# ufukpage/TripleD-Exploring-Depth-Estimation-with-Self-Supervised-Representation-Learning

Hardware: AMD Instinct MI355X
Metric: train imgs/sec at KITTI 192x640 bs=12/GPU (higher is better)
Workload: dtype bf16 convs (MFMA) + f32 loss kernels

## Files before the change

include/tripled_hip.h:

```cpp
#ifndef TRIPLED_HIP_H
#define TRIPLED_HIP_H

#include <stddef.h>
#include <stdint.h>

#ifdef __cplusplus
extern "C" {
#endif

#define TD_ABI_VERSION 3
#define TD_MAX_SRC 4

#define TD_OK 0
#define TD_ERR_BAD_ARG (-1)
#define TD_ERR_UNSUPPORTED (-2)
#define TD_ERR_LAUNCH (-3)
#define TD_ERR_WORKSPACE (-4)

typedef void* td_stream_t;

int td_abi_version(void);
const char* td_error_string(int code);
const char* td_last_hip_error(void);

// ... 113 lines not shown

int td_bn_partial_rows(long long M, int groups, int C);
int td_bn_fwd_partials(const void* x, int dtype, long long M, int groups, int C, float* partials, td_stream_t stream);
int td_bn_bwd_partials(const void* dy, const void* x, const void* y, int dtype, const float* gamma, const float* beta,
                       const float* save_mean, const float* save_invstd, int relu, long long M, int groups, int C, float* partials,
                       td_stream_t stream);
int td_bn_bwd_from_partials(const void* dy, const void* x, const void* y, int dtype, const float* gamma, const float* beta,
                            const float* save_mean, const float* save_invstd, int relu, long long M, int groups, int C,
                            float* partials, int stat_rows, void* dx, void* dresidual, float* dgamma, float* dbeta,
                            td_stream_t stream);
int td_conv1x1_fwd_bnrelu(const void* z, const void* w, long long M, int groups, int K, int N, float* in_partials, int in_rows,
                          const float* gamma, const float* beta, float* running_mean, float* running_var, float momentum, float eps,
                          float* save_mean, float* save_invstd, void* a_side, void* y, float* stat_partials, td_stream_t stream);
int td_conv1x1_dgrad(const void* dy, const void* w, long long M, int groups, int Cout, int Cin, const void* residual, void* dx,
                     td_stream_t stream);
int td_conv1x1_fwd_sum(const void* x, const void* w, long long M, int K, int N, const void* run_in, void* y, void* run_out,
                       td_stream_t stream);
int td_conv1x1_dgrad_bnsums(const void* dy, const void* w, long long M, int groups, int Cout, int Cin, const void* z,
                            const float* gamma, const float* beta, const float* save_mean, const float* save_invstd, void* dx,
                            float* out_partials, td_stream_t stream);
int td_conv1x1_dgrad_bnbwd(const void* g, const void* z, const void* w, long long M, int groups, int Cout, int Cin, float* in_partials,
                           int in_rows, const float* gamma, const float* beta, const float* save_mean, const float* save_invstd,
                           float* dgamma, float* dbeta, void* dz_side, const void* residual, void* dx, td_stream_t stream);

int td_bn_sync_fwd_sums(const void* x, int dtype, long long M, int groups, int C, float* sums, float* workspace,
                        td_stream_t stream);
int td_bn_sync_fwd_apply(const void* x, const void* residual, int dtype, const float* sums, const float* count,
                         const float* gamma, const float* beta, float* running_mean, float* running_var, float momentum,
                         float eps, int relu, long long M, int groups, int C, void* y, float* save_mean,
                         float* save_invstd, td_stream_t stream);
int td_bn_sync_bwd_sums(const void* dy, const void* x, const void* y, int dtype, const float* gamma, const float* beta,
                        const float* save_mean, const float* save_invstd, int relu, long long M, int groups, int C,
                        float* sums, float* workspace, td_stream_t stream);
int td_bn_sync_bwd_dx(const void* dy, const void* x, const void* y, int dtype, const float* local_sums,
                      const float* global_sums, const float* count, const float* gamma, const float* beta,
                      const float* save_mean, const float* save_invstd, int relu, long long M, int groups, int C,
                      void* dx, void* dresidual, float* dgamma, float* dbeta, float* coef, td_stream_t stream);

int td_edge_weights(const float* img, int B, int h, int w, float a, const float* scale6, float* Wt,
                    td_stream_t stream);
int td_featreg_num_blocks(int B, int h, int w, int C);
int td_featreg_fwd(const void* feat, int dtype, const float* Wt, int B, int h, int w, int C,
                   float* partial, td_stream_t stream);
int td_featreg_bwd(const void* feat, int dtype, const float* Wt, const float* gscale, int B, int h, int w,
                   int C, void* grad, td_stream_t stream);

// ... 106 lines not shown
```

tripled-exploring-depth-estimation-with-self-supervised-representation-learning_amd/csrc/td_conv1x1.hip:

```cpp
#include "td_conv_tile.h"

namespace td {

struct ConvRows {
  int Wo, HoWo, Wi, HiWi, stride;
};

__device__ __forceinline__ long long cv_src_row(long long m, const ConvRows& g) {
  if (g.stride == 1) return m;
  const long long b = m / g.HoWo;
  const int rem = (int)(m - b * g.HoWo);
  const int ho = rem / g.Wo, wo = rem - ho * g.Wo;
  return b * g.HiWi + (long long)ho * g.stride * g.Wi + (long long)wo * g.stride;
}

struct CvFuse {
  const __hip_bfloat16* a2;
  const float* part;
  int part_S, part_stride, part_rows;
  const float* gamma;
  const float* beta;
  float* mean;
  float* invstd;
  float* rmean;
// ... 33 lines not shown
    g0 = fmaf(z0, sc[2 * e], sh[2 * e]) <= 0.f ? 0.f : g0;
    g1 = fmaf(z1, sc[2 * e + 1], sh[2 * e + 1]) <= 0.f ? 0.f : g1;
    const float v0 = fmaf(k0[2 * e], g0, fmaf(k1[2 * e], z0, k2[2 * e]));
    const float v1 = fmaf(k0[2 * e + 1], g1, fmaf(k1[2 * e + 1], z1, k2[2 * e + 1]));
    o[e] = (unsigned)f2bf(v0) | ((unsigned)f2bf(v1) << 16);
  }
  return make_uint4(o[0], o[1], o[2], o[3]);
}

__device__ __forceinline__ void cv_sum_rows(const float* __restrict__ part, int S, int stride, int K, int c, float& A, float& B) {
  float2 v[CV_PRO_MAX_S];
#pragma unroll
  for (int u = 0; u < CV_PRO_MAX_S; ++u)
    v[u] = *reinterpret_cast<const float2*>(part + ((size_t)(u < S ? u : 0) * stride * K + c) * 2);
  A = 0.f;
  B = 0.f;
#pragma unroll
  for (int u = 0; u < CV_PRO_MAX_S; ++u) {
    A += u < S ? v[u].x : 0.f;
    B += u < S ? v[u].y : 0.f;
  }
}

template <int BM, int BN, bool BT, int PRO, int EPI, bool DEEP>
__global__ __launch_bounds__(CV_THREADS, 2) void conv1x1_mfma_kernel(
    const __hip_bfloat16* __restrict__ x, const __hip_bfloat16* __restrict__ w, __hip_bfloat16* __restrict__ y,
    float* __restrict__ ws, long long Mg, int K, int N, int tiles_per_group, int total_blocks, ConvRows geom, CvFuse fz) {
  using T = CvTile<BM, BN, BT>;
  constexpr int A_BYTES = T::A_BYTES, STAGE = T::STAGE, TN = T::TN, TM = T::TM;
  __shared__ __attribute__((aligned(16))) unsigned char lds[T::LDS_BYTES];
  __shared__ __attribute__((aligned(16))) float s_pro[PRO == 0 ? 4 : (PRO == 1 ? 2 : 5) * CV_PRO_MAX_K];

  const int tid = threadIdx.x, lane = tid & 63, wid = tid >> 6;
  const int wm = wid >> 1, wn = wid & 1, l31 = lane & 31, h = lane >> 5;

  const int L = cv_xcd_tile(blockIdx.x, total_blocks);
  const int NT = N / BN;
  const int nt = L % NT, mt = L / NT;
  const int grp = mt / tiles_per_group, s = mt - grp * tiles_per_group;
  const long long row0 = (long long)grp * Mg + (long long)s * BM;
  const int rows_valid = (int)((Mg - (long long)s * BM) < BM ? (Mg - (long long)s * BM) : BM);
  const int n0 = nt * BN;

  const int lc = tid & 7, lr = tid >> 3;
  constexpr int NA = BM / 32, NB = BN / 32;
  auto a_off = [&](int i) {
    int r = lr + 32 * i;
    r = r < rows_valid ? r : rows_valid - 1;
    return cv_src_row(row0 + r, geom) * (long long)K + lc * 8;
  };
  const long long oa0 = a_off(0), oa1 = a_off(1), oa2 = NA > 2 ? a_off(2) : oa0, oa3 = NA > 2 ? a_off(3) : oa0;
  const __hip_bfloat16 *pa0 = x + oa0, *pa1 = x + oa1, *pa2 = x + oa2, *pa3 = x + oa3;
  constexpr int CPR = BN / 8, RPP = CV_THREADS / CPR;
  const int bc = tid % CPR, br = tid / CPR;
  const __hip_bfloat16* pb0 = BT ? w + (long long)br * N + n0 + bc * 8 : w + (long long)(n0 + lr) * K + lc * 8;
  const long long bstep = BT ? (long long)RPP * N : 32ll * K;
  const __hip_bfloat16 *pb1 = pb0 + bstep, *pb2 = pb0 + (NB > 2 ? 2 : 0) * bstep, *pb3 = pb0 + (NB > 2 ? 3 : 0) * bstep;
  const long long bkt = BT ? (long long)CV_BK * N : (long long)CV_BK;
#define CV_DECL(S)                                                                          \
  uint4 ra0##S, ra1##S, ra2##S, ra3##S, rb0##S, rb1##S, rb2##S, rb3##S, rz0##S, rz1##S, rz2##S, rz3##S; \
  ra0##S = ra1##S = ra2##S = ra3##S = rb0##S = rb1##S = rb2##S = rb3##S = make_uint4(0, 0, 0, 0);       \
  rz0##S = rz1##S = rz2##S = rz3##S = make_uint4(0, 0, 0, 0);
  CV_DECL(A)
  CV_DECL(B)
#define CV_LD(p, kt) (*reinterpret_cast<const uint4*>((p) + (kt) * CV_BK))
#define CV_LDB(p, kt) (*reinterpret_cast<const uint4*>((p) + (kt) * bkt))
#define CV_LOAD_GLOBAL(kt, S)                                  \
  {                                                            \
    ra0##S = CV_LD(pa0, kt);                                   \
    ra1##S = CV_LD(pa1, kt);                                   \
    if (NA > 2) { ra2##S = CV_LD(pa2, kt); ra3##S = CV_LD(pa3, kt); } \
    if constexpr (PRO == 2) {                                  \
      rz0##S = CV_LD(fz.a2 + oa0, kt);                         \
      rz1##S = CV_LD(fz.a2 + oa1, kt);                         \
      if (NA > 2) { rz2##S = CV_LD(fz.a2 + oa2, kt); rz3##S = CV_LD(fz.a2 + oa3, kt); } \
    }                                                          \
    rb0##S = CV_LDB(pb0, kt);                                  \
    rb1##S = CV_LDB(pb1, kt);                                  \
    if (NB > 2) { rb2##S = CV_LDB(pb2, kt); rb3##S = CV_LDB(pb3, kt); } \
  }
#define CV_ST(base, i, v) (*reinterpret_cast<uint4*>((base) + cv_swz(lr + 32 * (i), lc)) = (v))
#define CV_STB(base, i, v)                                                                              \
  {                                                                                                     \
    if constexpr (BT) *reinterpret_cast<uint4*>((base) + (br + RPP * (i)) * T::PITCH_T + bc * 16) = (v); \
    else CV_ST(base, i, v);                                                                             \
  }
#define CV_PRO_A(kt, S)                                                                                 \
// ... 32 lines not shown
  }
#define CV_WRITE_LDS(stage, kt, S)                                       \
  {                                                                      \
    unsigned char* base_ = lds + (stage) * STAGE;                        \
    CV_PRO_A(kt, S)                                                      \
    CV_ST(base_, 0, ra0##S);                                             \
    CV_ST(base_, 1, ra1##S);                                             \
    if (NA > 2) { CV_ST(base_, 2, ra2##S); CV_ST(base_, 3, ra3##S); }    \
    CV_STB(base_ + A_BYTES, 0, rb0##S);                                  \
    CV_STB(base_ + A_BYTES, 1, rb1##S);                                  \
    if (NB > 2) { CV_STB(base_ + A_BYTES, 2, rb2##S); CV_STB(base_ + A_BYTES, 3, rb3##S); } \
  }

  CvAcc<BM, BN> acc;
#pragma unroll
  for (int i = 0; i < TN; ++i)
#pragma unroll
    for (int j = 0; j < TM; ++j)
#pragma unroll
      for (int e = 0; e < 16; ++e) acc.v[i][j][e] = 0.f;

  const int nk = K / CV_BK;
  CV_LOAD_GLOBAL(0, A)
  if constexpr (DEEP) CV_LOAD_GLOBAL(nk > 1 ? 1 : 0, B)

  if constexpr (PRO == 1) {
    const float* part = fz.part + (size_t)grp * fz.part_rows * K * 2;
    const bool first = (s == 0 && nt == 0);
    for (int c = tid; c < K; c += CV_THREADS) {
      float A, B;
      cv_sum_rows(part, fz.part_S, fz.part_stride, K, c, A, B);
      const double m = (double)A / (double)Mg;
      double var = (double)B / (double)Mg - m * m;
      var = var > 0.0 ? var : 0.0;
      const float mf = (float)m, isf = (float)(1.0 / sqrt(var + (double)fz.eps));
      const float scv = fz.gamma[c] * isf;
      s_pro[c] = scv;
      s_pro[CV_PRO_MAX_K + c] = fz.beta[c] - mf * scv;
      if (first) {
        fz.mean[(size_t)grp * K + c] = mf;
        fz.invstd[(size_t)grp * K + c] = isf;
      }
      if (fz.rmean && first && grp == 0) {
        double rm = fz.rmean[c], rv = fz.rvar[c];
        for (int g2 = 0; g2 < fz.G; ++g2) {
          float A2 = A, B2 = B;
          if (g2 != 0) cv_sum_rows(fz.part + (size_t)g2 * fz.part_rows * K * 2, fz.part_S, fz.part_stride, K, c, A2, B2);
// ... 23 lines not shown
      const float c1 = -c0 * is * dg * inv_m;
      s_pro[0 * CV_PRO_MAX_K + c] = c0;
      s_pro[1 * CV_PRO_MAX_K + c] = c1;
      s_pro[2 * CV_PRO_MAX_K + c] = -c0 * A * inv_m - c1 * mu;
      s_pro[3 * CV_PRO_MAX_K + c] = c0;
      s_pro[4 * CV_PRO_MAX_K + c] = fz.beta[c] - mu * c0;
      if (first) {
        float dg_tot = 0.f, db_tot = 0.f;
        for (int g2 = 0; g2 < fz.G; ++g2) {
          float A2 = A, B2 = B;
          if (g2 != 0) cv_sum_rows(fz.part + (size_t)g2 * fz.part_rows * K * 2, fz.part_S, fz.part_stride, K, c, A2, B2);
          dg_tot += B2 * fz.invstd[(size_t)g2 * K + c];
          db_tot += A2;
        }
        fz.dgamma[c] = dg_tot;
        fz.dbeta[c] = db_tot;
      }
    }
    __syncthreads();
  }

  CV_WRITE_LDS(0, 0, A)
  __syncthreads();
  if constexpr (!DEEP) {
    for (int kt = 0; kt < nk; ++kt) {
      const bool more = kt + 1 < nk;
      if (more) CV_LOAD_GLOBAL(kt + 1, A)
      const unsigned char* sa = lds + (kt & 1) * STAGE;
      cv_stage_mfma<BM, BN, BT>(acc, sa, sa + A_BYTES, wm, wn, l31, h);
      if (more) CV_WRITE_LDS((kt + 1) & 1, kt + 1, A)
      __syncthreads();
    }
  } else {
    const int last = nk - 1;
    for (int kt = 0; kt < nk; kt += 2) {
      const int k2 = kt + 2 < last ? kt + 2 : last, k1 = kt + 1 < last ? kt + 1 : last, k3 = kt + 3 < last ? kt + 3 : last;
      CV_LOAD_GLOBAL(k2, A)
      __builtin_amdgcn_sched_barrier(0);
      cv_stage_mfma<BM, BN, BT>(acc, lds, lds + A_BYTES, wm, wn, l31, h);
      CV_WRITE_LDS(1, k1, B)
      __syncthreads();
      if (kt + 1 >= nk) break;
      CV_LOAD_GLOBAL(k3, B)
      __builtin_amdgcn_sched_barrier(0);
      cv_stage_mfma<BM, BN, BT>(acc, lds + STAGE, lds + STAGE + A_BYTES, wm, wn, l31, h);
      CV_WRITE_LDS(0, k2, A)
      __syncthreads();
    }
  }

  CvEpi ep = fz.ep;
  if constexpr (EPI == 2) { ep.mean += (size_t)grp * N; ep.invstd += (size_t)grp * N; }
  cv_epilogue<BM, BN, EPI>(acc, lds, y, ws, row0, rows_valid, n0, N, (long long)grp * tiles_per_group + s, tid, wm, wn, l31, h, ep);
}

#undef CV_LOAD_GLOBAL
#undef CV_DECL
#undef CV_WRITE_LDS
#undef CV_PRO_A
#undef CV_LD
#undef CV_LDB
#undef CV_ST
#undef CV_STB

constexpr int WG_T = 64;
constexpr int WG_PITCH = WG_T * 2 + 64;

typedef __attribute__((ext_vector_type(4))) short cv_s16x4;

__device__ __forceinline__ cv_bf16x8 wg_frag(const unsigned char* tile, int col0, int ks, int lane) {
  const int g = lane >> 4, i = lane & 15;
  const int row = 16 * ks + 8 * (g >> 1) + (i >> 2);
  const unsigned char* p = tile + row * WG_PITCH + (col0 + 16 * (g & 1) + 4 * (i & 3)) * 2;
  typedef __attribute__((address_space(3))) cv_s16x4* lds_ptr;
  const cv_s16x4 lo = __builtin_amdgcn_ds_read_tr16_b64_v4i16((lds_ptr)(p));
  const cv_s16x4 hi = __builtin_amdgcn_ds_read_tr16_b64_v4i16((lds_ptr)(p + 4 * WG_PITCH));
  typedef __attribute__((ext_vector_type(8))) short s16x8;
  const s16x8 v = {lo[0], lo[1], lo[2], lo[3], hi[0], hi[1], hi[2], hi[3]};
  return __builtin_bit_cast(cv_bf16x8, v);
}

constexpr int WG_TILE_BYTES = WG_T * WG_PITCH, WG_STAGE = 2 * WG_TILE_BYTES, WG_LDS_BYTES = 2 * WG_STAGE;

__device__ __forceinline__ void wgrad_block(
    const __hip_bfloat16* __restrict__ dy, const __hip_bfloat16* __restrict__ x, float* __restrict__ part, long long M, int K, int N,
    int rows_per_split, int tiles_n, int tiles_k, ConvRows geom, int L, unsigned char* lds) {
  constexpr int TILE_BYTES = WG_TILE_BYTES, STAGE = WG_STAGE;
  const int tid = threadIdx.x, lane = tid & 63, wid = tid >> 6;
  const int wn = wid >> 1, wk = wid & 1;
  const int nt = L % tiles_n, kt = (L / tiles_n) % tiles_k, sp = L / (tiles_n * tiles_k);
  const int n0 = nt * WG_T, k0 = kt * WG_T;
  const long long m_lo = (long long)sp * rows_per_split;
  const long long m_hi = (m_lo + rows_per_split < M) ? m_lo + rows_per_split : M;
  const int nstage = (int)((m_hi - m_lo + WG_T - 1) / WG_T);

  const int lc = tid & 7, lr = tid >> 3;
  uint4 ry0a, ry1a, rx0a, rx1a, ry0b, ry1b, rx0b, rx1b;
#define WG_LOAD(st, S)                                                                                             \
  {                                                                                                                \
    const long long r0 = m_lo + (long long)(st) * WG_T + lr, r1 = r0 + 32;                                         \
    const uint4 z = make_uint4(0, 0, 0, 0);                                                                        \
    ry0##S = r0 < m_hi ? *reinterpret_cast<const uint4*>(dy + r0 * N + n0 + lc * 8) : z;                           \
    ry1##S = r1 < m_hi ? *reinterpret_cast<const uint4*>(dy + r1 * N + n0 + lc * 8) : z;                           \
    rx0##S = r0 < m_hi ? *reinterpret_cast<const uint4*>(x + cv_src_row(r0, geom) * (long long)K + k0 + lc * 8) : z; \
    rx1##S = r1 < m_hi ? *reinterpret_cast<const uint4*>(x + cv_src_row(r1, geom) * (long long)K + k0 + lc * 8) : z; \
  }
#define WG_WRITE(buf, S)                                                                         \
  {                                                                                              \
    unsigned char* b_ = lds + (buf) * STAGE;                                                     \
    *reinterpret_cast<uint4*>(b_ + lr * WG_PITCH + lc * 16) = ry0##S;                            \
    *reinterpret_cast<uint4*>(b_ + (lr + 32) * WG_PITCH + lc * 16) = ry1##S;                     \
    *reinterpret_cast<uint4*>(b_ + TILE_BYTES + lr * WG_PITCH + lc * 16) = rx0##S;               \
    *reinterpret_cast<uint4*>(b_ + TILE_BYTES + (lr + 32) * WG_PITCH + lc * 16) = rx1##S;        \
  }
#define WG_MFMA(buf)                                                                             \
  {                                                                                              \
    const unsigned char* ty = lds + (buf) * STAGE;                                               \
    const unsigned char* tx = ty + TILE_BYTES;                                                   \
    _Pragma("unroll") for (int ks = 0; ks < WG_T / 16; ++ks) {                                   \
      const cv_bf16x8 fa = wg_frag(ty, wn * 32, ks, lane);                  \
      const cv_bf16x8 fb = wg_frag(tx, wk * 32, ks, lane);                  \
      acc = __builtin_amdgcn_mfma_f32_32x32x16_bf16(fa, fb, acc, 0, 0, 0);                       \
    }                                                                                            \
  }
  cv_f32x16 acc;
#pragma unroll
  for (int e = 0; e < 16; ++e) acc[e] = 0.f;
  WG_LOAD(0, a)
  if (nstage > 1) WG_LOAD(1, b)
  WG_WRITE(0, a)
  __syncthreads();
  for (int st = 0; st < nstage; st += 2) {
    if (st + 2 < nstage) WG_LOAD(st + 2, a)
    WG_MFMA(0)
    if (st + 1 < nstage) WG_WRITE(1, b)
    __syncthreads();
    if (st + 1 >= nstage) break;
    if (st + 3 < nstage) WG_LOAD(st + 3, b)
    WG_MFMA(1)
    if (st + 2 < nstage) WG_WRITE(0, a)
    __syncthreads();
  }
#undef WG_MFMA
#undef WG_LOAD
#undef WG_WRITE
  float* out = part + ((size_t)sp * N + n0 + wn * 32 + 4 * (lane >> 5)) * K + k0 + wk * 32 + (lane & 31);
#pragma unroll
  for (int r = 0; r < 16; ++r) out[(size_t)((r & 3) + 8 * (r >> 2)) * K] = acc[r];
}

__global__ __launch_bounds__(CV_THREADS, 2) void conv1x1_wgrad_kernel(
    const __hip_bfloat16* __restrict__ dy, const __hip_bfloat16* __restrict__ x, float* __restrict__ part, long long M, int K, int N,
    int rows_per_split, int tiles_n, int tiles_k, ConvRows geom) {
  __shared__ __attribute__((aligned(16))) unsigned char lds[WG_LDS_BYTES];
  wgrad_block(dy, x, part, M, K, N, rows_per_split, tiles_n, tiles_k, geom, cv_xcd_tile(blockIdx.x, gridDim.x), lds);
}

constexpr int WG_GROUP_MAX = 40;
struct WgProblem {
  const __hip_bfloat16* dy;
  const __hip_bfloat16* x;
  float* part;
  long long M;
  int K, N, rows_per_split, tiles_n, tiles_k;
  ConvRows geom;
};
struct WgGroupArgs {
  WgProblem p[WG_GROUP_MAX];
  int first_block[WG_GROUP_MAX + 1];
  int n;
};
__global__ __launch_bounds__(CV_THREADS, 2) void conv1x1_wgrad_group_kernel(const WgGroupArgs a) {
  __shared__ __attribute__((aligned(16))) unsigned char lds[WG_LDS_BYTES];
  const int L = cv_xcd_tile(blockIdx.x, gridDim.x);
  int lo = 0, hi = a.n;
  while (hi - lo > 1) {
    const int mid = (lo + hi) >> 1;
    if (a.first_block[mid] <= L) lo = mid; else hi = mid;
  }
  const WgProblem& q = a.p[lo];
  wgrad_block(q.dy, q.x, q.part, q.M, q.K, q.N, q.rows_per_split, q.tiles_n, q.tiles_k, q.geom, L - a.first_block[lo], lds);
}

template <typename T>
__global__ __launch_bounds__(TD_THREADS) void conv1x1_wgrad_reduce_kernel(const float* __restrict__ part, int P, long long NK, T* __restrict__ dw) {
  __shared__ float4 red[16][16];
  const int c = threadIdx.x & 15, g = threadIdx.x >> 4;
  const long long i = ((long long)blockIdx.x * 16 + c) * 4;
  float4 a = make_float4(0.f, 0.f, 0.f, 0.f);
  if (i < NK) {
    for (int p = g; p < P; p += 16) {
      const float4 b = *reinterpret_cast<const float4*>(part + (size_t)p * NK + i);
      a.x += b.x; a.y += b.y; a.z += b.z; a.w += b.w;
    }
  }
  red[g][c] = a;
  __syncthreads();
  if (g == 0 && i < NK) {
#pragma unroll
    for (int j = 1; j < 16; ++j) {
      const float4 b = red[j][c];
      a.x += b.x; a.y += b.y; a.z += b.z; a.w += b.w;
    }
    if constexpr (sizeof(T) == 2) {
// ... 54 lines not shown
      *reinterpret_cast<float4*>(reinterpret_cast<float*>(q.dw) + i) = s4;
    }
  }
}

int cv_wgrad_reduce(const float* part, int P, long long NK, int dw_dtype, void* dw, hipStream_t st) {
  const unsigned blocks = (unsigned)((NK / 4 + 15) / 16);
  if (dw_dtype == TD_DTYPE_BF16)
    hipLaunchKernelGGL((conv1x1_wgrad_reduce_kernel<__hip_bfloat16>), dim3(blocks), dim3(TD_THREADS), 0, st, part, P, NK, (__hip_bfloat16*)dw);
  else
    hipLaunchKernelGGL((conv1x1_wgrad_reduce_kernel<float>), dim3(blocks), dim3(TD_THREADS), 0, st, part, P, NK, (float*)dw);
  return hipGetLastError() == hipSuccess ? TD_OK : TD_ERR_LAUNCH;
}

static inline int wg_splits(long long M, int K, int N) {
  const long long tiles = (long long)(N / WG_T) * (K / WG_T);
  long long p = (768 + tiles - 1) / tiles;
  const long long by_rows = (M + 4 * WG_T - 1) / (4 * WG_T);
  if (p > by_rows) p = by_rows;
  if (p > 512) p = 512;
  return (int)(p < 1 ? 1 : p);
}

template <int BM, int BN, bool BT, int PRO, int EPI, bool DEEP>
static int cv_launch(const void* x, const void* w, void* y, float* ws, long long Mg, int G, int K, int N, ConvRows geom, hipStream_t st,
                     const CvFuse& fz) {
  const int tpg = (int)((Mg + BM - 1) / BM);
  const long long nblk = (long long)G * tpg * (N / BN);
  if (nblk > 0x7fffffffll) return TD_ERR_UNSUPPORTED;
  hipLaunchKernelGGL((conv1x1_mfma_kernel<BM, BN, BT, PRO, EPI, DEEP>), dim3((unsigned)nblk), dim3(CV_THREADS), 0, st, (const __hip_bfloat16*)x,
                     (const __hip_bfloat16*)w, (__hip_bfloat16*)y, ws, Mg, K, N, tpg, (int)nblk, geom, fz);
  return hipGetLastError() == hipSuccess ? TD_OK : TD_ERR_LAUNCH;
}

template <bool BT, int PRO, int EPI>
static int cv_dispatch(const void* x, const void* w, void* y, float* ws, long long M, int G, int K, int N, ConvRows geom, hipStream_t st,
                       const CvFuse& fz) {
  const long long Mg = M / G;
  ConvTile t = cv_pick_tile(Mg, G, N);
  const bool deep = K >= 3 * CV_BK;
  if constexpr (PRO == 2) {
    if (t.bm == 128 && t.bn == 128) t.bn = 64;
  } else
    if (t.bm == 128 && t.bn == 128) return cv_launch<128, 128, BT, PRO, EPI, false>(x, w, y, ws, Mg, G, K, N, geom, st, fz);
  if (t.bm == 128 && t.bn == 64) {
    if constexpr (PRO == 0)
      if (deep) return cv_launch<128, 64, BT, PRO, EPI, true>(x, w, y, ws, Mg, G, K, N, geom, st, fz);
    return cv_launch<128, 64, BT, PRO, EPI, false>(x, w, y, ws, Mg, G, K, N, geom, st, fz);
  }
  if (deep) return cv_launch<64, 64, BT, PRO, EPI, true>(x, w, y, ws, Mg, G, K, N, geom, st, fz);
  return cv_launch<64, 64, BT, PRO, EPI, false>(x, w, y, ws, Mg, G, K, N, geom, st, fz);
}

}

static bool cv_shape_ok(long long M, int G, int K, int N) {
  return M > 0 && G >= 1 && G <= 64 && M % G == 0 && K > 0 && N > 0 && K % 64 == 0 && N % 64 == 0;
}

extern "C" int td_conv1x1_stat_rows(long long M, int groups, int N) {
  if (M <= 0 || groups < 1 || M % groups != 0 || N <= 0 || N % 64 != 0) return 0;
  const td::ConvTile t = td::cv_pick_tile(M / groups, groups, N);
  return (int)((M / groups + t.bm - 1) / t.bm);
}

extern "C" int td_conv1x1_fwd(const void* x, const void* w, long long M, int groups, int K, int N, int Hi, int Wi, int stride, void* y,
                              float* stat_partials, td_stream_t stream) {
  if (!x || !w || !y || !cv_shape_ok(M, groups, K, N) || stride < 1) return TD_ERR_BAD_ARG;
  td::ConvRows geom = {0, 0, 0, 0, 1};
  if (stride > 1) {
    if (Hi <= 0 || Wi <= 0) return TD_ERR_BAD_ARG;
    const int Ho = (Hi - 1) / stride + 1, Wo = (Wi - 1) / stride + 1;
    if (M % ((long long)Ho * Wo) != 0) return TD_ERR_BAD_ARG;
    geom = {Wo, Ho * Wo, Wi, Hi * Wi, stride};
  }
  if (M * (long long)(K > N ? K : N) >= (1ll << 40)) return TD_ERR_UNSUPPORTED;
  return td::cv_dispatch<false, 0, 0>(x, w, y, stat_partials, M, groups, K, N, geom, (hipStream_t)stream, td::CvFuse{});
}

namespace td {
// ... 72 lines not shown
extern "C" long long td_conv1x1_wgrad_workspace_floats(long long M, int K, int N) {
  if (M <= 0 || K <= 0 || N <= 0 || K % 64 != 0 || N % 64 != 0) return 0;
  return (long long)td::wg_splits(M, K, N) * N * K;
}

extern "C" int td_conv1x1_wgrad(const void* dy, const void* x, long long M, int K, int N, int Hi, int Wi, int stride, int dw_dtype,
                                void* dw, float* workspace, td_stream_t stream) {
  if (!dy || !x || !dw || !workspace || M <= 0 || K <= 0 || N <= 0 || K % 64 != 0 || N % 64 != 0 || stride < 1) return TD_ERR_BAD_ARG;
  if (dw_dtype != TD_DTYPE_BF16 && dw_dtype != TD_DTYPE_F32) return TD_ERR_UNSUPPORTED;
  td::ConvRows geom = {0, 0, 0, 0, 1};
  if (stride > 1) {
    if (Hi <= 0 || Wi <= 0) return TD_ERR_BAD_ARG;
    const int Ho = (Hi - 1) / stride + 1, Wo = (Wi - 1) / stride + 1;
    if (M % ((long long)Ho * Wo) != 0) return TD_ERR_BAD_ARG;
    geom = {Wo, Ho * Wo, Wi, Hi * Wi, stride};
  }
  if (M * (long long)(K > N ? K : N) >= (1ll << 40)) return TD_ERR_UNSUPPORTED;
  hipStream_t st = (hipStream_t)stream;
  const int P = td::wg_splits(M, K, N);
  long long rps = (M + P - 1) / P;
  rps = (rps + td::WG_T - 1) / td::WG_T * td::WG_T;
  const int P_eff = (int)((M + rps - 1) / rps);
  const int tn = N / td::WG_T, tk = K / td::WG_T;
  hipLaunchKernelGGL(td::conv1x1_wgrad_kernel, dim3((unsigned)(tn * tk * P_eff)), dim3(td::CV_THREADS), 0, st, (const __hip_bfloat16*)dy,
                     (const __hip_bfloat16*)x, workspace, M, K, N, (int)rps, tn, tk, geom);
  const long long NK = (long long)N * K;
  const unsigned blocks = (unsigned)((NK / 4 + 15) / 16);
  if (dw_dtype == TD_DTYPE_BF16)
    hipLaunchKernelGGL((td::conv1x1_wgrad_reduce_kernel<__hip_bfloat16>), dim3(blocks), dim3(TD_THREADS), 0, st, (const float*)workspace, P_eff,
                       NK, (__hip_bfloat16*)dw);
  else
    hipLaunchKernelGGL((td::conv1x1_wgrad_reduce_kernel<float>), dim3(blocks), dim3(TD_THREADS), 0, st, (const float*)workspace, P_eff, NK,
                       (float*)dw);
  return hipGetLastError() == hipSuccess ? TD_OK : TD_ERR_LAUNCH;
}

extern "C" int td_conv1x1_wgrad_group(int n, const void* const* dy, const void* const* x, const long long* M, const int* K, const int* N,
                                      const int* Hi, const int* Wi, const int* stride, const int* dw_dtype, void* const* dw,
                                      float* const* workspace, td_stream_t stream) {
  if (n < 0 || (n > 0 && (!dy || !x || !M || !K || !N || !Hi || !Wi || !stride || !dw_dtype || !dw || !workspace))) return TD_ERR_BAD_ARG;
  hipStream_t st = (hipStream_t)stream;
  for (int i = 0; i < n; ++i) {
    if (!dy[i] || !x[i] || !dw[i] || !workspace[i] || M[i] <= 0 || K[i] <= 0 || N[i] <= 0 || K[i] % 64 != 0 || N[i] % 64 != 0 || stride[i] < 1)
      return TD_ERR_BAD_ARG;
    if (dw_dtype[i] != TD_DTYPE_BF16 && dw_dtype[i] != TD_DTYPE_F32) return TD_ERR_UNSUPPORTED;
    if (M[i] * (long long)(K[i] > N[i] ? K[i] : N[i]) >= (1ll << 40)) return TD_ERR_UNSUPPORTED;
    if (stride[i] > 1) {
      if (Hi[i] <= 0 || Wi[i] <= 0) return TD_ERR_BAD_ARG;
      const int Ho = (Hi[i] - 1) / stride[i] + 1, Wo = (Wi[i] - 1) / stride[i] + 1;
      if (M[i] % ((long long)Ho * Wo) != 0) return TD_ERR_BAD_ARG;
    }
  }
  int P_eff[4096];
  if (n > 4096) return TD_ERR_UNSUPPORTED;
  for (int base = 0; base < n; base += td::WG_GROUP_MAX) {
    td::WgGroupArgs a;
    a.n = n - base < td::WG_GROUP_MAX ? n - base : td::WG_GROUP_MAX;
    long long blocks = 0;
    for (int j = 0; j < a.n; ++j) {
      const int i = base + j;
      td::ConvRows geom = {0, 0, 0, 0, 1};
      if (stride[i] > 1) {
        const int Ho = (Hi[i] - 1) / stride[i] + 1, Wo = (Wi[i] - 1) / stride[i] + 1;
        geom = {Wo, Ho * Wo, Wi[i], Hi[i] * Wi[i], stride[i]};
      }
      const int P = td::wg_splits(M[i], K[i], N[i]);
      long long rps = (M[i] + P - 1) / P;
      rps = (rps + td::WG_T - 1) / td::WG_T * td::WG_T;
      P_eff[i] = (int)((M[i] + rps - 1) / rps);
      td::WgProblem& q = a.p[j];
      q.dy = (const __hip_bfloat16*)dy[i]; q.x = (const __hip_bfloat16*)x[i]; q.part = workspace[i]; q.M = M[i]; q.K = K[i]; q.N = N[i];
      q.rows_per_split = (int)rps; q.tiles_n = N[i] / td::WG_T; q.tiles_k = K[i] / td::WG_T; q.geom = geom;
      a.first_block[j] = (int)blocks;
      blocks += (long long)q.tiles_n * q.tiles_k * P_eff[i];
      if (blocks > 0x7fffffffll) return TD_ERR_UNSUPPORTED;
    }
    for (int j = a.n; j <= td::WG_GROUP_MAX; ++j) a.first_block[j] = (int)blocks;
    hipLaunchKernelGGL(td::conv1x1_wgrad_group_kernel, dim3((unsigned)blocks), dim3(td::CV_THREADS), 0, st, a);
  }
  for (int base = 0; base < n; base += td::RD_GROUP_MAX) {
    td::RdGroupArgs a;
    a.n = n - base < td::RD_GROUP_MAX ? n - base : td::RD_GROUP_MAX;
    long long blocks = 0;
    for (int j = 0; j < a.n; ++j) {
      const int i = base + j;
      td::RdProblem& q = a.p[j];
      q.part = workspace[i]; q.dw = dw[i]; q.NK = (long long)N[i] * K[i]; q.P = P_eff[i]; q.bf16 = dw_dtype[i] == TD_DTYPE_BF16;
      a.first_block[j] = (int)blocks;
      blocks += (q.NK / 4 + 15) / 16;
    }
    for (int j = a.n; j <= td::RD_GROUP_MAX; ++j) a.first_block[j] = (int)blocks;
    hipLaunchKernelGGL(td::conv1x1_wgrad_reduce_group_kernel, dim3((unsigned)blocks), dim3(TD_THREADS), 0, st, a);
  }
  return hipGetLastError() == hipSuccess ? TD_OK : TD_ERR_LAUNCH;
}
```

tripled-exploring-depth-estimation-with-self-supervised-representation-learning_amd/native.py:

```python
import ctypes
import os

import torch

from . import dispatch

_HERE = os.path.dirname(os.path.abspath(__file__))
LIB_PATH = os.path.join(_HERE, "lib", "libtripled_hip.so")

TD_MAX_SRC = 4

_PTRARR = ctypes.POINTER(ctypes.c_void_p)
_I, _F, _P = ctypes.c_int, ctypes.c_float, ctypes.c_void_p
_LLARR = ctypes.POINTER(ctypes.c_longlong)
_IARR = ctypes.POINTER(ctypes.c_int)
ABI_VERSION = 3

SIGNATURES = {
    "td_abi_version": (_I, []),
    "td_error_string": (ctypes.c_char_p, [_I]),
    "td_last_hip_error": (ctypes.c_char_p, []),
    "td_photo_num_blocks": (_I, [_I, _I, _I]),
    "td_photo_bwd_num_blocks": (_I, [_I, _I, _I]),
    "td_photo_identity": (_I, [_P, _PTRARR, _I, _I, _I, _I, _P, _P, _PTRARR, _P]),
# ... 23 lines not shown
    "td_bn_fwd": (_I, [_P, _P, _I, _P, _P, _P, _P, _F, _F, _I, ctypes.c_longlong, _I, _I, _P, _P, _P, _P, _P]),
    "td_conv1x1_stat_rows": (_I, [ctypes.c_longlong, _I, _I]),
    "td_conv1x1_fwd": (_I, [_P, _P, ctypes.c_longlong, _I, _I, _I, _I, _I, _I, _P, _P, _P]),
    "td_conv3x3_fwd": (_I, [_P, _P, _I, _I, _I, _I, _I, _I, _I, _I, _P, _P, _P]),
    "td_conv3x3_wgrad_workspace_floats": (ctypes.c_longlong, [_I, _I, _I, _I, _I]),
    "td_conv3x3_wgrad": (_I, [_P, _P, _I, _I, _I, _I, _I, _I, _I, _P, _P, _P]),
    "td_conv1x1_wgrad_workspace_floats": (ctypes.c_longlong, [ctypes.c_longlong, _I, _I]),
    "td_conv1x1_wgrad": (_I, [_P, _P, ctypes.c_longlong, _I, _I, _I, _I, _I, _I, _P, _P, _P]),
    "td_conv1x1_wgrad_group": (_I, [_I, _PTRARR, _PTRARR, _LLARR, _IARR, _IARR, _IARR, _IARR, _IARR, _IARR, _PTRARR, _PTRARR, _P]),
    "td_bn_fwd_from_partials": (_I, [_P, _P, _I, _P, _P, _P, _P, _F, _F, _I, ctypes.c_longlong, _I, _I, _P, _I, _P, _P, _P, _P]),
    "td_bias_act_workspace_floats": (ctypes.c_longlong, [ctypes.c_longlong, _I]),
    "td_bias_act_fwd": (_I, [_P, _P, _I, _I, ctypes.c_longlong, _I, _I, _P, _P]),
    "td_bias_act_bwd": (_I, [_P, _P, _I, ctypes.c_longlong, _I, _I, _P, _P, _I, _P, _P]),
    "td_gather_flat": (_I, [_PTRARR, _LLARR, _LLARR, _I, _I, _P, _P]),
    "td_adam_flat": (_I, [_P, _P, _P, _P, _P, ctypes.c_longlong, ctypes.c_longlong, _P, _P, _F, ctypes.c_double, ctypes.c_double, _F, _P, _F, _P]),
    "td_bn_partial_rows": (_I, [ctypes.c_longlong, _I, _I]),
    "td_bn_fwd_partials": (_I, [_P, _I, ctypes.c_longlong, _I, _I, _P, _P]),
    "td_bn_bwd_partials": (_I, [_P, _P, _P, _I, _P, _P, _P, _P, _I, ctypes.c_longlong, _I, _I, _P, _P]),
    "td_bn_bwd_from_partials": (_I, [_P, _P, _P, _I, _P, _P, _P, _P, _I, ctypes.c_longlong, _I, _I, _P, _I, _P, _P, _P, _P, _P]),
    "td_conv1x1_fwd_bnrelu": (_I, [_P, _P, ctypes.c_longlong, _I, _I, _I, _P, _I, _P, _P, _P, _P, _F, _F, _P, _P, _P, _P, _P, _P]),
    "td_conv1x1_dgrad": (_I, [_P, _P, ctypes.c_longlong, _I, _I, _I, _P, _P, _P]),
    "td_conv1x1_dgrad_bnsums": (_I, [_P, _P, ctypes.c_longlong, _I, _I, _I, _P, _P, _P, _P, _P, _P, _P, _P]),
    "td_conv1x1_dgrad_bnbwd": (_I, [_P, _P, _P, ctypes.c_longlong, _I, _I, _I, _P, _I, _P, _P, _P, _P, _P, _P, _P, _P, _P, _P]),
    "td_bn_bwd": (_I, [_P, _P, _P, _I, _P, _P, _P, _P, _I, ctypes.c_longlong, _I, _I, _P, _P, _P, _P, _P, _P]),
    "td_edge_weights": (_I, [_P, _I, _I, _I, _F, ctypes.POINTER(ctypes.c_float), _P, _P]),
    "td_featreg_num_blocks": (_I, [_I, _I, _I, _I]),
    "td_featreg_fwd": (_I, [_P, _I, _P, _I, _I, _I, _I, _P, _P]),
    "td_featreg_bwd": (_I, [_P, _I, _P, _P, _I, _I, _I, _I, _P, _P]),
    "td_recon_num_tasks": (_I, [_I, _I, _I]),
    "td_recon_fwd": (_I, [_P, _P, _P, _I, _I, _I, _P, _P]),
    "td_recon_bwd": (_I, [_P, _P, _P, _P, _I, _I, _I, _P, _P]),
    "td_reflpad1_fwd": (_I, [_P, _I, _I, _I, _I, _I, _P, _P]),
    "td_reflpad1_bwd": (_I, [_P, _I, _I, _I, _I, _I, _P, _P]),
    "td_up2_reflpad1_fwd": (_I, [_P, _I, _I, _I, _I, _I, _P, _P]),
    "td_up2_reflpad1_bwd": (_I, [_P, _I, _I, _I, _I, _I, _P, _P]),
    "td_featwarp_num_blocks": (_I, [_I, _I, _I]),
    "td_featwarp_fwd": (_I, [_P, _PTRARR, _I, _I, _P, _P, _P, _I, _I, _I, _I, _I, _I, _F, _F, _P, _P, _P]),
    "td_featwarp_bwd": (_I, [_P, _PTRARR, _I, _I, _P, _P, _P, _P, _P, _F, _I, _I, _I, _I, _I, _I, _F, _F, _P, _PTRARR,
                             _P, _P, _P]),
    "td_featwarp_dsrc_finish": (_I, [_P, _P, _F, _I, ctypes.c_longlong, _I, _P, _P]),
    "td_reduce_partials": (_I, [_P, _I, _I, _I, _P, _P]),
    "td_bn_sync_fwd_sums": (_I, [_P, _I, ctypes.c_longlong, _I, _I, _P, _P, _P]),
    "td_bn_sync_fwd_apply": (_I, [_P, _P, _I, _P, _P, _P, _P, _P, _P, _F, _F, _I, ctypes.c_longlong, _I, _I, _P, _P, _P, _P]),
    "td_bn_sync_bwd_sums": (_I, [_P, _P, _P, _I, _P, _P, _P, _P, _I, ctypes.c_longlong, _I, _I, _P, _P, _P]),
    "td_bn_sync_bwd_dx": (_I, [_P, _P, _P, _I, _P, _P, _P, _P, _P, _P, _P, _I, ctypes.c_longlong, _I, _I, _P, _P, _P, _P, _P, _P]),
    "td_fp8_num_blocks": (_I, [ctypes.c_longlong]),
# ... 151 lines not shown
```

Baseline: 444.5.

## Add depth-4 global-load prefetch pipeline to 1x1 conv forward and wgrad kernels

Generalises the 1x1 conv MFMA kernel's prefetch from a boolean deep mode to a depth template (1, 2 or 4). A four-register-stage rotation keeps more global loads in flight ahead of the MFMA stages. Depth 4 is chosen for 64x64 tiles with long K and few blocks, and for wgrad kernels with enough output tiles; an env var and API cap allow overriding. The aim is to hide memory latency in low-occupancy, long-K convolutions, at the cost of more live registers (risking spills or lower occupancy) and extra template instantiations.

```diff
diff --git a/include/tripled_hip.h b/include/tripled_hip.h
--- a/include/tripled_hip.h
+++ b/include/tripled_hip.h
@@ -159,6 +159,8 @@
 int td_conv1x1_dgrad_bnbwd(const void* g, const void* z, const void* w, long long M, int groups, int Cout, int Cin, float* in_partials,
                            int in_rows, const float* gamma, const float* beta, const float* save_mean, const float* save_invstd,
                            float* dgamma, float* dbeta, void* dz_side, const void* residual, void* dx, td_stream_t stream);
+#define TD_CONV1X1_DEPTH_FORCE 0x100
+int td_conv1x1_prefetch_depth(int cap);
 
 int td_bn_sync_fwd_sums(const void* x, int dtype, long long M, int groups, int C, float* sums, float* workspace,
                         td_stream_t stream);
diff --git a/tripled-exploring-depth-estimation-with-self-supervised-representation-learning_amd/csrc/td_conv1x1.hip b/tripled-exploring-depth-estimation-with-self-supervised-representation-learning_amd/csrc/td_conv1x1.hip
--- a/tripled-exploring-depth-estimation-with-self-supervised-representation-learning_amd/csrc/td_conv1x1.hip
+++ b/tripled-exploring-depth-estimation-with-self-supervised-representation-learning_amd/csrc/td_conv1x1.hip
@@ -1,3 +1,6 @@
+#include <atomic>
+#include <cstdlib>
+
 #include "td_conv_tile.h"
 
 namespace td {
@@ -79,7 +82,7 @@
   }
 }
 
-template <int BM, int BN, bool BT, int PRO, int EPI, bool DEEP>
+template <int BM, int BN, bool BT, int PRO, int EPI, int DEPTH>
 __global__ __launch_bounds__(CV_THREADS, 2) void conv1x1_mfma_kernel(
     const __hip_bfloat16* __restrict__ x, const __hip_bfloat16* __restrict__ w, __hip_bfloat16* __restrict__ y,
     float* __restrict__ ws, long long Mg, int K, int N, int tiles_per_group, int total_blocks, ConvRows geom, CvFuse fz) {
@@ -120,6 +123,8 @@
   rz0##S = rz1##S = rz2##S = rz3##S = make_uint4(0, 0, 0, 0);
   CV_DECL(A)
   CV_DECL(B)
+  CV_DECL(C)
+  CV_DECL(D)
 #define CV_LD(p, kt) (*reinterpret_cast<const uint4*>((p) + (kt) * CV_BK))
 #define CV_LDB(p, kt) (*reinterpret_cast<const uint4*>((p) + (kt) * bkt))
 #define CV_LOAD_GLOBAL(kt, S)                                  \
@@ -198,7 +203,11 @@
 
   const int nk = K / CV_BK;
   CV_LOAD_GLOBAL(0, A)
-  if constexpr (DEEP) CV_LOAD_GLOBAL(nk > 1 ? 1 : 0, B)
+  if constexpr (DEPTH >= 2) CV_LOAD_GLOBAL(nk > 1 ? 1 : 0, B)
+  if constexpr (DEPTH == 4) {
+    CV_LOAD_GLOBAL(nk > 2 ? 2 : nk - 1, C)
+    CV_LOAD_GLOBAL(nk > 3 ? 3 : nk - 1, D)
+  }
 
   if constexpr (PRO == 1) {
     const float* part = fz.part + (size_t)grp * fz.part_rows * K * 2;
@@ -268,7 +277,7 @@
 
   CV_WRITE_LDS(0, 0, A)
   __syncthreads();
-  if constexpr (!DEEP) {
+  if constexpr (DEPTH == 1) {
     for (int kt = 0; kt < nk; ++kt) {
       const bool more = kt + 1 < nk;
       if (more) CV_LOAD_GLOBAL(kt + 1, A)
@@ -277,7 +286,7 @@
       if (more) CV_WRITE_LDS((kt + 1) & 1, kt + 1, A)
       __syncthreads();
     }
-  } else {
+  } else if constexpr (DEPTH == 2) {
     const int last = nk - 1;
     for (int kt = 0; kt < nk; kt += 2) {
       const int k2 = kt + 2 < last ? kt + 2 : last, k1 = kt + 1 < last ? kt + 1 : last, k3 = kt + 3 < last ? kt + 3 : last;
@@ -293,6 +302,37 @@
       CV_WRITE_LDS(0, k2, A)
       __syncthreads();
     }
+  } else {
+    static_assert(DEPTH == 4, "prefetch depth is 1, 2 or 4");
+    const int last = nk - 1;
+#define CV_STEP(i, SL, SW)                                                                          \
+  {                                                                                                  \
+    const int kl_ = kt + (i) + 4 < last ? kt + (i) + 4 : last, kw_ = kt + (i) + 1 < last ? kt + (i) + 1 : last; \
+    CV_LOAD_GLOBAL(kl_, SL)                                                                          \
+    __builtin_amdgcn_sched_barrier(0);                                                               \
+    cv_stage_mfma<BM, BN, BT>(acc, lds + ((i) & 1) * STAGE, lds + ((i) & 1) * STAGE + A_BYTES, wm, wn, l31, h); \
+    __builtin_amdgcn_sched_barrier(0);                                                               \
+    CV_WRITE_LDS(((i) + 1) & 1, kw_, SW)                                                             \
+    __syncthreads();                                                                                 \
+    __builtin_amdgcn_sched_barrier(0);                                                               \
+  }
+    int kt = 0;
+    {
+      for (; kt + 4 <= nk; kt += 4) {
+        CV_STEP(0, A, B)
+        CV_STEP(1, B, C)
+        CV_STEP(2, C, D)
+        CV_STEP(3, D, A)
+      }
+      if (kt < nk) {
+        CV_STEP(0, A, B)
+        if (kt + 1 < nk) {
+          CV_STEP(1, B, C)
+          if (kt + 2 < nk) CV_STEP(2, C, D)
+        }
+      }
+    }
+#undef CV_STEP
   }
 
   CvEpi ep = fz.ep;
@@ -326,8 +366,11 @@
   return __builtin_bit_cast(cv_bf16x8, v);
 }
 
+__device__ __forceinline__ uint4 wg_keep(uint4 v, unsigned mask) { return make_uint4(v.x & mask, v.y & mask, v.z & mask, v.w & mask); }
+
 constexpr int WG_TILE_BYTES = WG_T * WG_PITCH, WG_STAGE = 2 * WG_TILE_BYTES, WG_LDS_BYTES = 2 * WG_STAGE;
 
+template <int DEPTH>
 __device__ __forceinline__ void wgrad_block(
     const __hip_bfloat16* __restrict__ dy, const __hip_bfloat16* __restrict__ x, float* __restrict__ part, long long M, int K, int N,
     int rows_per_split, int tiles_n, int tiles_k, ConvRows geom, int L, unsigned char* lds) {
@@ -372,20 +415,65 @@
   cv_f32x16 acc;
 #pragma unroll
   for (int e = 0; e < 16; ++e) acc[e] = 0.f;
-  WG_LOAD(0, a)
-  if (nstage > 1) WG_LOAD(1, b)
-  WG_WRITE(0, a)
-  __syncthreads();
-  for (int st = 0; st < nstage; st += 2) {
-    if (st + 2 < nstage) WG_LOAD(st + 2, a)
-    WG_MFMA(0)
-    if (st + 1 < nstage) WG_WRITE(1, b)
+  if constexpr (DEPTH == 2) {
+    WG_LOAD(0, a)
+    if (nstage > 1) WG_LOAD(1, b)
+    WG_WRITE(0, a)
     __syncthreads();
-    if (st + 1 >= nstage) break;
-    if (st + 3 < nstage) WG_LOAD(st + 3, b)
-    WG_MFMA(1)
-    if (st + 2 < nstage) WG_WRITE(0, a)
+    for (int st = 0; st < nstage; st += 2) {
+      if (st + 2 < nstage) WG_LOAD(st + 2, a)
+      WG_MFMA(0)
+      if (st + 1 < nstage) WG_WRITE(1, b)
+      __syncthreads();
+      if (st + 1 >= nstage) break;
+      if (st + 3 < nstage) WG_LOAD(st + 3, b)
+      WG_MFMA(1)
+      if (st + 2 < nstage) WG_WRITE(0, a)
+      __syncthreads();
+    }
+  } else {
+    static_assert(DEPTH == 4, "prefetch depth is 2 or 4");
+    uint4 ry0c, ry1c, rx0c, rx1c, ry0d, ry1d, rx0d, rx1d;
+#define WG_LOAD4(st, S)                                                                                            \
+  {                                                                                                                \
+    const long long r0 = m_lo + (long long)(st) * WG_T + lr, r1 = r0 + 32;                                         \
+    const long long c0 = r0 < m_hi ? r0 : m_hi - 1, c1 = r1 < m_hi ? r1 : m_hi - 1;                                \
+    const unsigned k0_ = r0 < m_hi ? 0xffffffffu : 0u, k1_ = r1 < m_hi ? 0xffffffffu : 0u;                         \
+    ry0##S = wg_keep(*reinterpret_cast<const uint4*>(dy + c0 * N + n0 + lc * 8), k0_);                             \
+    ry1##S = wg_keep(*reinterpret_cast<const uint4*>(dy + c1 * N + n0 + lc * 8), k1_);                             \
+    rx0##S = wg_keep(*reinterpret_cast<const uint4*>(x + cv_src_row(c0, geom) * (long long)K + k0 + lc * 8), k0_); \
+    rx1##S = wg_keep(*reinterpret_cast<const uint4*>(x + cv_src_row(c1, geom) * (long long)K + k0 + lc * 8), k1_); \
+  }
+#define WG_STEP4(i, SL, SW)                         \
+  {                                                 \
+    WG_LOAD4(st + (i) + 4, SL)                      \
+    __builtin_amdgcn_sched_barrier(0);              \
+    WG_MFMA((i) & 1)                                \
+    WG_WRITE(((i) + 1) & 1, SW)                     \
+    __syncthreads();                                \
+  }
+    WG_LOAD4(0, a)
+    WG_LOAD4(1, b)
+    WG_LOAD4(2, c)
+    WG_LOAD4(3, d)
+    WG_WRITE(0, a)
     __syncthreads();
+    int st = 0;
+    for (; st + 4 <= nstage; st += 4) {
+      WG_STEP4(0, a, b)
+      WG_STEP4(1, b, c)
+      WG_STEP4(2, c, d)
+      WG_STEP4(3, d, a)
+    }
+    if (st < nstage) {
+      WG_STEP4(0, a, b)
+      if (st + 1 < nstage) {
+        WG_STEP4(1, b, c)
+        if (st + 2 < nstage) WG_STEP4(2, c, d)
+      }
+    }
+#undef WG_STEP4
+#undef WG_LOAD4
   }
 #undef WG_MFMA
 #undef WG_LOAD
@@ -395,11 +483,12 @@
   for (int r = 0; r < 16; ++r) out[(size_t)((r & 3) + 8 * (r >> 2)) * K] = acc[r];
 }
 
+template <int DEPTH>
 __global__ __launch_bounds__(CV_THREADS, 2) void conv1x1_wgrad_kernel(
     const __hip_bfloat16* __restrict__ dy, const __hip_bfloat16* __restrict__ x, float* __restrict__ part, long long M, int K, int N,
     int rows_per_split, int tiles_n, int tiles_k, ConvRows geom) {
   __shared__ __attribute__((aligned(16))) unsigned char lds[WG_LDS_BYTES];
-  wgrad_block(dy, x, part, M, K, N, rows_per_split, tiles_n, tiles_k, geom, cv_xcd_tile(blockIdx.x, gridDim.x), lds);
+  wgrad_block<DEPTH>(dy, x, part, M, K, N, rows_per_split, tiles_n, tiles_k, geom, cv_xcd_tile(blockIdx.x, gridDim.x), lds);
 }
 
 constexpr int WG_GROUP_MAX = 40;
@@ -409,6 +498,7 @@
   float* part;
   long long M;
   int K, N, rows_per_split, tiles_n, tiles_k;
+  int depth;
   ConvRows geom;
 };
 struct WgGroupArgs {
@@ -416,6 +506,7 @@
   int first_block[WG_GROUP_MAX + 1];
   int n;
 };
+template <int DEPTH>
 __global__ __launch_bounds__(CV_THREADS, 2) void conv1x1_wgrad_group_kernel(const WgGroupArgs a) {
   __shared__ __attribute__((aligned(16))) unsigned char lds[WG_LDS_BYTES];
   const int L = cv_xcd_tile(blockIdx.x, gridDim.x);
@@ -425,7 +516,10 @@
     if (a.first_block[mid] <= L) lo = mid; else hi = mid;
   }
   const WgProblem& q = a.p[lo];
-  wgrad_block(q.dy, q.x, q.part, q.M, q.K, q.N, q.rows_per_split, q.tiles_n, q.tiles_k, q.geom, L - a.first_block[lo], lds);
+  if (DEPTH == 4 && q.depth == 4)
+    wgrad_block<4>(q.dy, q.x, q.part, q.M, q.K, q.N, q.rows_per_split, q.tiles_n, q.tiles_k, q.geom, L - a.first_block[lo], lds);
+  else
+    wgrad_block<2>(q.dy, q.x, q.part, q.M, q.K, q.N, q.rows_per_split, q.tiles_n, q.tiles_k, q.geom, L - a.first_block[lo], lds);
 }
 
 template <typename T>
@@ -526,15 +620,40 @@
   return (int)(p < 1 ? 1 : p);
 }
 
-template <int BM, int BN, bool BT, int PRO, int EPI, bool DEEP>
+template <int BM, int BN, bool BT, int PRO, int EPI, int DEPTH>
 static int cv_launch(const void* x, const void* w, void* y, float* ws, long long Mg, int G, int K, int N, ConvRows geom, hipStream_t st,
                      const CvFuse& fz) {
   const int tpg = (int)((Mg + BM - 1) / BM);
   const long long nblk = (long long)G * tpg * (N / BN);
   if (nblk > 0x7fffffffll) return TD_ERR_UNSUPPORTED;
-  hipLaunchKernelGGL((conv1x1_mfma_kernel<BM, BN, BT, PRO, EPI, DEEP>), dim3((unsigned)nblk), dim3(CV_THREADS), 0, st, (const __hip_bfloat16*)x,
+  hipLaunchKernelGGL((conv1x1_mfma_kernel<BM, BN, BT, PRO, EPI, DEPTH>), dim3((unsigned)nblk), dim3(CV_THREADS), 0, st, (const __hip_bfloat16*)x,
                      (const __hip_bfloat16*)w, (__hip_bfloat16*)y, ws, Mg, K, N, tpg, (int)nblk, geom, fz);
   return hipGetLastError() == hipSuccess ? TD_OK : TD_ERR_LAUNCH;
+}
+
+static bool cv_depth_cap_ok(int cap) { return cap == 0 || cap == 1 || cap == 2 || cap == 4 || cap == (4 | TD_CONV1X1_DEPTH_FORCE); }
+static std::atomic<int>& cv_depth_cap() {
+  static std::atomic<int> cap{[] {
+    const char* e = getenv("TD_CONV1X1_DEPTH");
+    const int v = e ? atoi(e) : 0;
+    return cv_depth_cap_ok(v) ? v : 0;
+  }()};
+  return cap;
+}
+constexpr int CV_D4_MIN_NK = 32, CV_D4_MAX_BLOCKS = 256;
+static int cv_depth(int bm, int pro, int nk, long long blocks) {
+  int d = nk >= 3 ? 2 : 1;
+  if (bm == 128 && pro != 0) d = 1;
+  const int cap = cv_depth_cap().load(std::memory_order_relaxed);
+  if (bm == 64 && pro == 0 && (cap == (4 | TD_CONV1X1_DEPTH_FORCE) || (nk >= CV_D4_MIN_NK && blocks <= CV_D4_MAX_BLOCKS))) d = 4;
+  if (cap == 1 || cap == 2) d = d < cap ? d : cap;
+  return d;
+}
+static int wg_depth(int K, int N) {
+  const int cap = cv_depth_cap().load(std::memory_order_relaxed);
+  if (cap == 1 || cap == 2) return 2;
+  if (cap == (4 | TD_CONV1X1_DEPTH_FORCE)) return 4;
+  return (long long)(N / WG_T) * (K / WG_T) >= 16 ? 4 : 2;
 }
 
 template <bool BT, int PRO, int EPI>
@@ -542,24 +661,31 @@
                        const CvFuse& fz) {
   const long long Mg = M / G;
   ConvTile t = cv_pick_tile(Mg, G, N);
-  const bool deep = K >= 3 * CV_BK;
   if constexpr (PRO == 2) {
     if (t.bm == 128 && t.bn == 128) t.bn = 64;
   } else
-    if (t.bm == 128 && t.bn == 128) return cv_launch<128, 128, BT, PRO, EPI, false>(x, w, y, ws, Mg, G, K, N, geom, st, fz);
+    if (t.bm == 128 && t.bn == 128) return cv_launch<128, 128, BT, PRO, EPI, 1>(x, w, y, ws, Mg, G, K, N, geom, st, fz);
+  const int depth = cv_depth(t.bm, PRO, K / CV_BK, (long long)G * ((Mg + t.bm - 1) / t.bm) * (N / t.bn));
   if (t.bm == 128 && t.bn == 64) {
     if constexpr (PRO == 0)
-      if (deep) return cv_launch<128, 64, BT, PRO, EPI, true>(x, w, y, ws, Mg, G, K, N, geom, st, fz);
-    return cv_launch<128, 64, BT, PRO, EPI, false>(x, w, y, ws, Mg, G, K, N, geom, st, fz);
-  }
-  if (deep) return cv_launch<64, 64, BT, PRO, EPI, true>(x, w, y, ws, Mg, G, K, N, geom, st, fz);
-  return cv_launch<64, 64, BT, PRO, EPI, false>(x, w, y, ws, Mg, G, K, N, geom, st, fz);
+      if (depth == 2) return cv_launch<128, 64, BT, PRO, EPI, 2>(x, w, y, ws, Mg, G, K, N, geom, st, fz);
+    return cv_launch<128, 64, BT, PRO, EPI, 1>(x, w, y, ws, Mg, G, K, N, geom, st, fz);
+  }
+  if constexpr (PRO == 0)
+    if (depth == 4) return cv_launch<64, 64, BT, PRO, EPI, 4>(x, w, y, ws, Mg, G, K, N, geom, st, fz);
+  if (depth == 2) return cv_launch<64, 64, BT, PRO, EPI, 2>(x, w, y, ws, Mg, G, K, N, geom, st, fz);
+  return cv_launch<64, 64, BT, PRO, EPI, 1>(x, w, y, ws, Mg, G, K, N, geom, st, fz);
 }
 
 }
 
 static bool cv_shape_ok(long long M, int G, int K, int N) {
   return M > 0 && G >= 1 && G <= 64 && M % G == 0 && K > 0 && N > 0 && K % 64 == 0 && N % 64 == 0;
+}
+
+extern "C" int td_conv1x1_prefetch_depth(int cap) {
+  if (!td::cv_depth_cap_ok(cap)) return TD_ERR_BAD_ARG;
+  return td::cv_depth_cap().exchange(cap);
 }
 
 extern "C" int td_conv1x1_stat_rows(long long M, int groups, int N) {
@@ -678,8 +804,12 @@
   rps = (rps + td::WG_T - 1) / td::WG_T * td::WG_T;
   const int P_eff = (int)((M + rps - 1) / rps);
   const int tn = N / td::WG_T, tk = K / td::WG_T;
-  hipLaunchKernelGGL(td::conv1x1_wgrad_kernel, dim3((unsigned)(tn * tk * P_eff)), dim3(td::CV_THREADS), 0, st, (const __hip_bfloat16*)dy,
-                     (const __hip_bfloat16*)x, workspace, M, K, N, (int)rps, tn, tk, geom);
+  if (td::wg_depth(K, N) == 4)
+    hipLaunchKernelGGL(td::conv1x1_wgrad_kernel<4>, dim3((unsigned)(tn * tk * P_eff)), dim3(td::CV_THREADS), 0, st, (const __hip_bfloat16*)dy,
+                       (const __hip_bfloat16*)x, workspace, M, K, N, (int)rps, tn, tk, geom);
+  else
+    hipLaunchKernelGGL(td::conv1x1_wgrad_kernel<2>, dim3((unsigned)(tn * tk * P_eff)), dim3(td::CV_THREADS), 0, st, (const __hip_bfloat16*)dy,
+                       (const __hip_bfloat16*)x, workspace, M, K, N, (int)rps, tn, tk, geom);
   const long long NK = (long long)N * K;
   const unsigned blocks = (unsigned)((NK / 4 + 15) / 16);
   if (dw_dtype == TD_DTYPE_BF16)
@@ -713,6 +843,7 @@
     td::WgGroupArgs a;
     a.n = n - base < td::WG_GROUP_MAX ? n - base : td::WG_GROUP_MAX;
     long long blocks = 0;
+    bool any4 = false;
     for (int j = 0; j < a.n; ++j) {
       const int i = base + j;
       td::ConvRows geom = {0, 0, 0, 0, 1};
@@ -727,12 +858,17 @@
       td::WgProblem& q = a.p[j];
       q.dy = (const __hip_bfloat16*)dy[i]; q.x = (const __hip_bfloat16*)x[i]; q.part = workspace[i]; q.M = M[i]; q.K = K[i]; q.N = N[i];
       q.rows_per_split = (int)rps; q.tiles_n = N[i] / td::WG_T; q.tiles_k = K[i] / td::WG_T; q.geom = geom;
+      q.depth = td::wg_depth(K[i], N[i]);
+      any4 = any4 || q.depth == 4;
       a.first_block[j] = (int)blocks;
       blocks += (long long)q.tiles_n * q.tiles_k * P_eff[i];
       if (blocks > 0x7fffffffll) return TD_ERR_UNSUPPORTED;
     }
     for (int j = a.n; j <= td::WG_GROUP_MAX; ++j) a.first_block[j] = (int)blocks;
-    hipLaunchKernelGGL(td::conv1x1_wgrad_group_kernel, dim3((unsigned)blocks), dim3(td::CV_THREADS), 0, st, a);
+    if (any4)
+      hipLaunchKernelGGL(td::conv1x1_wgrad_group_kernel<4>, dim3((unsigned)blocks), dim3(td::CV_THREADS), 0, st, a);
+    else
+      hipLaunchKernelGGL(td::conv1x1_wgrad_group_kernel<2>, dim3((unsigned)blocks), dim3(td::CV_THREADS), 0, st, a);
   }
   for (int base = 0; base < n; base += td::RD_GROUP_MAX) {
     td::RdGroupArgs a;
diff --git a/tripled-exploring-depth-estimation-with-self-supervised-representation-learning_amd/native.py b/tripled-exploring-depth-estimation-with-self-supervised-representation-learning_amd/native.py
--- a/tripled-exploring-depth-estimation-with-self-supervised-representation-learning_amd/native.py
+++ b/tripled-exploring-depth-estimation-with-self-supervised-representation-learning_amd/native.py
@@ -69,6 +69,7 @@
     "td_conv1x1_dgrad": (_I, [_P, _P, ctypes.c_longlong, _I, _I, _I, _P, _P, _P]),
     "td_conv1x1_dgrad_bnsums": (_I, [_P, _P, ctypes.c_longlong, _I, _I, _I, _P, _P, _P, _P, _P, _P, _P, _P]),
     "td_conv1x1_dgrad_bnbwd": (_I, [_P, _P, _P, ctypes.c_longlong, _I, _I, _I, _P, _I, _P, _P, _P, _P, _P, _P, _P, _P, _P, _P]),
+    "td_conv1x1_prefetch_depth": (_I, [_I]),
     "td_bn_bwd": (_I, [_P, _P, _P, _I, _P, _P, _P, _P, _I, ctypes.c_longlong, _I, _I, _P, _P, _P, _P, _P, _P]),
     "td_edge_weights": (_I, [_P, _I, _I, _I, _F, ctypes.POINTER(ctypes.c_float), _P, _P]),
     "td_featreg_num_blocks": (_I, [_I, _I, _I, _I]),
```

Measured after the change: 447.5 (median of 2 runs). Within noise of the previous version (+0.7%).
